# Pixie8888/R3DFSSeg

Hardware: AMD Instinct MI355X
Metric: episodes/sec S3DIS 2-way 5-shot 2048-pt (MPTI+attention, train step: forward+backward+grad all-reduce+Adam) (higher is better)
Workload: dtype f32 (index-free GEMMs -- self-attention, 1x1 convolutions, weight gradients, the EdgeConv backward's edge GEMMs -- as bf16x3 split products on the bf16 MFMA with fp32 accumulate; every index-deciding result: fp32)

## Files before the change

r3dfsseg_amd/csrc/knn.hip:

```cpp
#include <stdlib.h>
#include "common.h"

#define KNN_Q 32
#define KNN_CH 128
#define KNN_SLAB 64
#define KNN_ROWS_PER_WAVE 8

enum { R3D_SCORE_DGCNN = 0, R3D_SCORE_L2 = 1 };

__global__ void r3d_sqnorm_kernel(const float* __restrict__ x, long ldx, int rows, int C,
                                  float* __restrict__ out) {
  int i = blockIdx.x * blockDim.x + threadIdx.x;
  if (i >= rows) return;
  const float* p = x + (long)i * ldx;
  float acc = 0.f;
  for (int c = 0; c < C; ++c) acc = __builtin_fmaf(p[c], p[c], acc);
  out[i] = acc;
}

template <int R>
struct TopList {
  float v[R];
  int id[R];
};
// ... 359 lines not shown
        const unsigned long long ge = __ballot(lv[r] >= cv);
        const int p = h ? __popc((unsigned)(ge >> 32)) : __popc((unsigned)ge);
        const float upv = dpp_wave_shr1_f(lv[r]);
        const int upi = dpp_wave_shr1_i(li[r]);
        if (act) {
          if (j == p) { lv[r] = cv; li[r] = cidx; }
          else if (j > p) { lv[r] = upv; li[r] = upi; }
        }
        const float tlo = r3d_readlane_f(lv[r], klo);
        const float thi = r3d_readlane_f(lv[r], khi);
        thr[r] = h ? thi : tlo;
      }
    }
  };
  {
    int st = w;
    if (st < nsub) bload(st, bfA, njA);
    while (st < nsub) {
      const int st2 = st + 4;
      if (st2 < nsub) bload(st2, bfB, njB);
      {
        f32x16 sc;
        scores(st, bfA, njA, sc);
        select(st, sc);
      }
      st = st2;
      if (st >= nsub) break;
      const int st3 = st + 4;
      if (st3 < nsub) bload(st3, bfA, njA);
      {
        f32x16 sc;
        scores(st, bfB, njB, sc);
        select(st, sc);
      }
      st = st3;
    }
  }
  KSTAMP(3);

  __syncthreads();
  float* mv = smem;
  int* mi = (int*)(smem + 32 * 128);
#pragma unroll
  for (int r = 0; r < 16; ++r) {
    const int q = r3d_acc_row(r, lane);
    mv[(q * 4 + w) * 32 + j] = lv[r];
    mi[(q * 4 + w) * 32 + j] = li[r];
  }
  __syncthreads();
  for (int qq = 0; qq < 8; ++qq) {
    const int q = 8 * w + qq;
    const int row = q0 + q;
    if (row >= n) break;
    const float v0 = mv[q * 128 + lane], v1 = mv[q * 128 + 64 + lane];
    const int i0 = mi[q * 128 + lane], i1 = mi[q * 128 + 64 + lane];
    int rank0 = 0, rank1 = 0;
#pragma unroll
    for (int l4 = 0; l4 < 4; ++l4) {
      const float lvv = (l4 < 2) ? v0 : v1;
      const int lii = (l4 < 2) ? i0 : i1;
      const unsigned long long real = __ballot(lvv != -INFINITY);
      const int cnt = __popc((unsigned)(real >> (32 * (l4 & 1))));
      for (int t = 0; t < cnt; ++t) {
        const float ov = r3d_readlane_f(lvv, 32 * (l4 & 1) + t);
        const int oi = __builtin_amdgcn_readlane(lii, 32 * (l4 & 1) + t);
        rank0 += entry_better(ov, oi, v0, i0) ? 1 : 0;
        rank1 += entry_better(ov, oi, v1, i1) ? 1 : 0;
      }
    }
    if (v0 != -INFINITY && rank0 < k) {
      idx_out[((long)b * N + row) * k + rank0] = i0;
      if (score_out) score_out[((long)b * N + row) * k + rank0] = v0;
    }
    if (v1 != -INFINITY && rank1 < k) {
      idx_out[((long)b * N + row) * k + rank1] = i1;
      if (score_out) score_out[((long)b * N + row) * k + rank1] = v1;
    }
  }
  KSTAMP(4);
}

static __device__ __forceinline__ unsigned knn_lane_xor(unsigned v, int j, int lane) {
  const int x = (int)v;
  switch (j) {
    case 1: return (unsigned)__builtin_amdgcn_update_dpp(x, x, 0xB1, 0xF, 0xF, false);
    case 2: return (unsigned)__builtin_amdgcn_update_dpp(x, x, 0x4E, 0xF, 0xF, false);
    case 4: {
      const int t = __builtin_amdgcn_update_dpp(x, x, 0x104, 0xF, 0x5, false);
      return (unsigned)__builtin_amdgcn_update_dpp(t, x, 0x114, 0xF, 0xA, false);
    }
    case 8: return (unsigned)__builtin_amdgcn_update_dpp(x, x, 0x128, 0xF, 0xF, false);
    case 16: {
      const auto r = __builtin_amdgcn_permlane16_swap(v, v, false, false);
      return (lane & 16) ? r[0] : r[1];
    }
    default: {
      const auto r = __builtin_amdgcn_permlane32_swap(v, v, false, false);
      return (lane & 32) ? r[0] : r[1];
    }
  }
}

template <int R>
static __device__ __forceinline__ void knn_bitonic_desc(unsigned (&khi)[R], unsigned (&klo)[R], int lane) {
  static_assert(R == 1 || R == 2 || R == 4 || R == 8, "a power of two");
#pragma unroll
  for (int k = 2; k <= 64 * R; k <<= 1) {
#pragma unroll
    for (int j = k >> 1; j > 0; j >>= 1) {
      if (j >= 64) {
        const int dj = j >> 6;
#pragma unroll
        for (int i = 0; i < R; ++i) {
          if (i & dj) continue;
          const bool desc = ((64 * i) & k) == 0;
          const unsigned long long a = ((unsigned long long)khi[i] << 32) | klo[i];
          const unsigned long long b = ((unsigned long long)khi[i + dj] << 32) | klo[i + dj];
          const bool swap = desc ? a < b : a > b;
          const unsigned ah = khi[i], al = klo[i];
          khi[i] = swap ? khi[i + dj] : ah; klo[i] = swap ? klo[i + dj] : al;
          khi[i + dj] = swap ? ah : khi[i + dj]; klo[i + dj] = swap ? al : klo[i + dj];
        }
      } else {
        const bool lower = (lane & j) == 0;
#pragma unroll
        for (int i = 0; i < R; ++i) {
          const bool desc = (((64 * i) | lane) & k) == 0;
          const unsigned oh = knn_lane_xor(khi[i], j, lane), ol = knn_lane_xor(klo[i], j, lane);
          const unsigned long long a = ((unsigned long long)khi[i] << 32) | klo[i];
          const unsigned long long b = ((unsigned long long)oh << 32) | ol;
          const bool take = (lower == desc) ? b > a : b < a;
          khi[i] = take ? oh : khi[i];
          klo[i] = take ? ol : klo[i];
        }
      }
    }
  }
}

template <int KB_WAVES, int KB_CAP, int KB_TOP, int KCH ,
          int KB_SAMPLE ,
          bool FULLC ,
          int SMODE ,
          bool BFA ,
          bool BFB = false >
__global__ __launch_bounds__(64 * KB_WAVES) __attribute__((amdgpu_waves_per_eu(KB_WAVES == 4 && (FULLC || KCH < 32) ? 3 : 2)))
void r3d_knn_append_kernel(
    const float* __restrict__ xT, long ldT, int N, int C, int k, int mode, const int* __restrict__ n_dev, int n_dev_stride,
    const float* __restrict__ nrm, int* __restrict__ idx_out, float* __restrict__ score_out,
    int* __restrict__ status, int* __restrict__ tile_flags, int nsplit, int* __restrict__ idx_tmp,
    float* __restrict__ sc_tmp, const unsigned short* __restrict__ xpk ,
    const float* __restrict__ cnorm ,
    const float* __restrict__ xpm , long ldx) {
  static_assert(!BFA || (KCH == 32 && FULLC), "the bf16 threshold pass takes whole 64-channel chunks");
  static_assert(!BFB || BFA, "the bf16 filter pass shares the threshold pass's pieces");
  constexpr int KB_GROUPS = KB_WAVES * 32;
  const int z = blockIdx.z;
  extern __shared__ __attribute__((aligned(16))) float smem[];
  __shared__ int cnt_s[32];
  __shared__ float tau_s[32];
  const int lin = r3d_xcd_swizzle((int)(blockIdx.y * gridDim.x + blockIdx.x), (int)(gridDim.x * gridDim.y));
  const int b = lin / (int)gridDim.x, tile_x = lin - b * (int)gridDim.x;
  const int n = n_dev ? min(n_dev[(long)b * n_dev_stride], N) : N;
  const int q0 = tile_x * 32;
  if (q0 >= n) return;
  const int tid = threadIdx.x, lane = tid & 63, w = tid >> 6;
  const int h = lane >> 5, j = lane & 31;
  const int nch = (C + 2 * KCH - 1) / (2 * KCH);
  const int Cs = nch * 2 * KCH + (BFB ? 4 : 1);
  float* Aq = smem;
  float* region = smem + 32 * Cs;
  const float* xb = xT + (long)b * C * ldT;
  const float* nb = nrm + (long)b * N;

  for (int e = tid; e < 32 * nch * 2 * KCH; e += 64 * KB_WAVES) {
    const int c = e >> 5, jj = e & 31;
    const float v = xb[(long)min(c, C - 1) * ldT + min(q0 + jj, n - 1)];
    Aq[jj * Cs + c] = r3d_keep(v, c < C && q0 + jj < n);
  }
  if (tid < 32) cnt_s[tid] = 0;
  const int Cp = nch * 64;
  const int QRS = 2 * Cp + 8;
  unsigned short* Aqb = reinterpret_cast<unsigned short*>(region + ((32 * (KB_TOP * KB_GROUPS + 1) + 3) & ~3));
  const unsigned short* xpb = BFA ? xpk + (long)b * N * 2 * Cp : nullptr;
  if (BFA) {
    const int cpr = 2 * Cp / 8;
    for (int e = tid; e < 32 * cpr; e += 64 * KB_WAVES) {
      const int c8 = e >> 5, jj = e & 31;
      *reinterpret_cast<r3d_u32x4*>(Aqb + jj * QRS + 8 * c8) =
          *reinterpret_cast<const r3d_u32x4*>(xpb + ((long)c8 * N + min(q0 + jj, n - 1)) * 8);
    }
  }
  KSTAMP(8);
  float nq[16];
#pragma unroll
  for (int r = 0; r < 16; ++r) {
    const int row = q0 + r3d_acc_row(r, lane);
    nq[r] = r3d_keep(nb[min(row, n - 1)], row < n);
  }
  const float* cnb = BFA ? cnorm + (long)b * N : nullptr;
  const float slack = (float)(C + 8) * 0x1p-24f;
  auto bound_k = [&](int i) { return cnb[i] * (1.f + 0x1p-12f) + nb[i] * slack; };
  float* kq_s = reinterpret_cast<float*>(Aqb + 32 * QRS);
  if (BFA && tid < 32) kq_s[tid] = bound_k(min(q0 + tid, n - 1));
  auto bound_ku = [&](int i) { return cnb[i] * (1.f - 0x1p-12f) - nb[i] * slack; };
  if (BFB && tid < 32) kq_s[32 + tid] = bound_ku(min(q0 + tid, n - 1));
  __syncthreads();

  const int nsub = ((n + 31) / 32 - z + nsplit - 1) / nsplit;
  const int my_sub = (nsub - w + KB_WAVES - 1) / KB_WAVES;
  const int T = (w < nsub) ? my_sub * nch : 0;

  int stride = KB_SAMPLE;
  auto bload = [&](int t, float (&bf)[KCH]) {
    const int st = (w + KB_WAVES * stride * (t / nch)) * nsplit + z, ch = (t % nch);
    const int cand = 32 * st + j;
    const bool ok = cand < n;
    const int cc = min(cand, n - 1);
    if (FULLC) {
      const float* p = xb + (long)(2 * KCH * ch + h) * ldT + cc;
      const long st2 = 2 * ldT;
#pragma unroll
      for (int s = 0; s < KCH; ++s) bf[s] = p[s * st2];
    } else {
#pragma unroll
      for (int s = 0; s < KCH; ++s) {
        const int c = 2 * KCH * ch + 2 * s + h;
        bf[s] = r3d_keep(xb[(long)min(c, C - 1) * ldT + cc], ok && c < C);
      }
    }
  };
  f32x16 acc;
  auto mma = [&](int t, const float (&bf)[KCH]) {
    const int ch = (t % nch);
    if (ch == 0) {
#pragma unroll
      for (int r = 0; r < 16; ++r) acc[r] = 0.f;
    }
    const float* ap = Aq + j * Cs + 2 * KCH * ch + h;
    float av[KCH];
#pragma unroll
    for (int s = 0; s < KCH; ++s) av[s] = ap[2 * s];
    __builtin_amdgcn_sched_barrier(0);
#pragma unroll
    for (int s = 0; s < KCH; ++s) acc = __builtin_amdgcn_mfma_f32_32x32x2f32(av[s], bf[s], acc, 0, 0, 0);
  };
  float kb[16];
  auto load_kb = [&](int which) {
#pragma unroll
    for (int r = 0; r < 16; ++r) kb[r] = kq_s[32 * which + r3d_acc_row(r, lane)];
  };
  auto scores_lb = [&](int st, f32x16& sc) {
    const int cand = 32 * st + j;
    const float kj = bound_k(min(cand, n - 1));
#pragma unroll
    for (int r = 0; r < 16; ++r) {
      const float v = __builtin_fmaf(2.f, acc[r], -(kb[r] + kj));
      sc[r] = SMODE == R3D_SCORE_DGCNN ? v : fminf(v, 0.f);
    }
    if (32 * st + 32 > n) {
      const bool valid = cand < n;
#pragma unroll
      for (int r = 0; r < 16; ++r) sc[r] = valid ? sc[r] : -INFINITY;
    }
  };
  auto scores_ub = [&](int st, f32x16& sc) {
    const int cand = 32 * st + j;
    const float kj = bound_ku(min(cand, n - 1));
#pragma unroll
    for (int r = 0; r < 16; ++r) {
      const float v = __builtin_fmaf(2.f, acc[r], -(kb[r] + kj));
      sc[r] = SMODE == R3D_SCORE_DGCNN ? v : fminf(v, 0.f);
    }
    if (32 * st + 32 > n) {
      const bool valid = cand < n;
#pragma unroll
      for (int r = 0; r < 16; ++r) sc[r] = valid ? sc[r] : -INFINITY;
    }
  };
  auto scores = [&](int st, f32x16& sc) {
    const int cand = 32 * st + j;
    const bool valid = cand < n;
    const float nj = r3d_keep(nb[min(cand, n - 1)], valid);
#pragma unroll
    for (int r = 0; r < 16; ++r) {
      float v;
      if (SMODE == R3D_SCORE_DGCNN) {
        const float inner = -2.f * acc[r];
        v = ((-nj) - inner) - nq[r];
      } else {
        const float dis = (nq[r] + nj) - 2.f * acc[r];
        v = -fmaxf(dis, 0.f);
      }
      sc[r] = v;
    }
    if (32 * st + 32 > n) {
#pragma unroll
      for (int r = 0; r < 16; ++r) sc[r] = valid ? sc[r] : -INFINITY;
    }
  };

  float bfA[KCH], bfB[KCH];
  float g1[16], g2[16];
#pragma unroll
  for (int r = 0; r < 16; ++r) { g1[r] = -INFINITY; g2[r] = -INFINITY; }
  auto finishA_sub = [&](int i) {
    f32x16 sc;
    if (BFA) scores_lb((w + KB_WAVES * stride * i) * nsplit + z, sc);
    else scores((w + KB_WAVES * stride * i) * nsplit + z, sc);
#pragma unroll
    for (int r = 0; r < 16; ++r) {
      const float x = sc[r];
      if (KB_TOP == 2) {
        const float lo = fminf(g1[r], x);
        g2[r] = fmaxf(g2[r], lo);
      }
      g1[r] = fmaxf(g1[r], x);
    }
  };
  auto finishA = [&](int t) {
    if ((t % nch) == nch - 1) finishA_sub(t / nch);
  };
  KSTAMP(9);
  const int TA = (w < nsub) ? ((my_sub + KB_SAMPLE - 1) / KB_SAMPLE) * nch : 0;
  r3d_u32x4 pfA[8], pfB[8];
  const __amdgpu_buffer_rsrc_t rpk = __builtin_amdgcn_make_buffer_rsrc(
      (void*)(BFA ? xpb : (const unsigned short*)xT), 0, BFA ? (int)((long)N * 2 * Cp * 2) : 0, 0x00020000);
  const int chunk_b = N * 16;
  auto pload = [&](int i, int ch, r3d_u32x4 (&pf)[8]) {
    const int st = (w + KB_WAVES * stride * i) * nsplit + z;
    const int cc = min(32 * st + j, n - 1);
    const int voff = (h * N + cc) * 16;
    const int soff = 8 * ch * chunk_b, lo = (Cp / 8) * chunk_b;
#pragma unroll
    for (int s4 = 0; s4 < 4; ++s4) {
      pf[2 * s4] = __builtin_amdgcn_raw_buffer_load_b128(rpk, voff, soff + 2 * s4 * chunk_b, 0);
      pf[2 * s4 + 1] = __builtin_amdgcn_raw_buffer_load_b128(rpk, voff, soff + lo + 2 * s4 * chunk_b, 0);
    }
  };
  auto pmma = [&](int ch, const r3d_u32x4 (&pf)[8]) {
    if (ch == 0) {
#pragma unroll
      for (int r = 0; r < 16; ++r) acc[r] = 0.f;
    }
    const unsigned short* ap = Aqb + j * QRS + 64 * ch + 8 * h;
#pragma unroll
    for (int half = 0; half < 2; ++half) {
      r3d_u32x4 ah[2], al[2];
#pragma unroll
      for (int u = 0; u < 2; ++u) {
        ah[u] = *reinterpret_cast<const r3d_u32x4*>(ap + 16 * (2 * half + u));
        al[u] = *reinterpret_cast<const r3d_u32x4*>(ap + Cp + 16 * (2 * half + u));
      }
#pragma unroll
      for (int u = 0; u < 2; ++u) {
        const int s4 = 2 * half + u;
        acc = r3d_mfma_bf16(al[u], pf[2 * s4], acc);
        acc = r3d_mfma_bf16(ah[u], pf[2 * s4 + 1], acc);
        acc = r3d_mfma_bf16(ah[u], pf[2 * s4], acc);
      }
    }
  };
  auto bf_pass = [&](int n_sub, auto&& finish) {
    const int U = n_sub * nch;
    if (U <= 0) return;
    int i_c = 0, ch_c = 0, i_n = 0, ch_n = 0;
    auto advance = [&](int& i, int& ch) {
      if (++ch == nch) { ch = 0; ++i; }
    };
    pload(0, 0, pfA);
    advance(i_n, ch_n);
    int u = 0;
    for (; u + 1 < U; u += 2) {
      pload(i_n, ch_n, pfB);
      __builtin_amdgcn_sched_barrier(0);
      pmma(ch_c, pfA);
      if (ch_c == nch - 1) finish(i_c);
      i_c = i_n; ch_c = ch_n;
      advance(i_n, ch_n);
      const bool more = u + 2 < U;
      pload(more ? i_n : i_c, more ? ch_n : ch_c, pfA);
      __builtin_amdgcn_sched_barrier(0);
      pmma(ch_c, pfB);
      if (ch_c == nch - 1) finish(i_c);
      i_c = i_n; ch_c = ch_n;
      advance(i_n, ch_n);
    }
    if (u < U) {
      pmma(ch_c, pfA);
      if (ch_c == nch - 1) finish(i_c);
    }
  };
  if (BFA) {
    load_kb(0);
    bf_pass((w < nsub) ? (my_sub + KB_SAMPLE - 1) / KB_SAMPLE : 0, finishA_sub);
  } else {
    if (TA > 0) bload(0, bfB);
    for (int t = 0; t < TA; ++t) {
#pragma unroll
      for (int s = 0; s < KCH; ++s) bfA[s] = bfB[s];
      if (t + 1 < TA) bload(t + 1, bfB);
      __builtin_amdgcn_sched_barrier(0);
      mma(t, bfA);
      finishA(t);
    }
  }
  KSTAMP(10);
  stride = 1;
  {
    constexpr int GS = KB_TOP * KB_GROUPS + 1;
#pragma unroll
    for (int r = 0; r < 16; ++r) {
      const int q = r3d_acc_row(r, lane);
      region[q * GS + KB_TOP * (32 * w + j)] = g1[r];
      if (KB_TOP == 2) region[q * GS + 2 * (32 * w + j) + 1] = g2[r];
    }
    __syncthreads();
    for (int qq = 0; qq < 32 / KB_WAVES; ++qq) {
      const int q = (32 / KB_WAVES) * w + qq;
      unsigned key[KB_TOP * KB_GROUPS / 64];
#pragma unroll
      for (int i = 0; i < KB_TOP * KB_GROUPS / 64; ++i) key[i] = f2key(region[q * GS + 64 * i + lane]) >> 16;
      unsigned res = 0;
      for (int bit = 15; bit >= 0; --bit) {
        const unsigned cand = res | (1u << bit);
        int c = 0;
#pragma unroll
        for (int i = 0; i < KB_TOP * KB_GROUPS / 64; ++i) c += __popcll(__ballot(key[i] >= cand));
        if (c >= k) res = cand;
      }
      if (lane == 0) tau_s[q] = key2f(res << 16);
    }
    __syncthreads();
  }
  KSTAMP(11);
  float tauq[16];
#pragma unroll
  for (int r = 0; r < 16; ++r) tauq[r] = q0 + r3d_acc_row(r, lane) < n ? tau_s[r3d_acc_row(r, lane)] : INFINITY;
  __syncthreads();

  static_assert(!BFB || 32 * KB_CAP <= 32 * (KB_TOP * KB_GROUPS + 1), "the index buffer must end in front of the query pieces");
  float* bufv = region + (BFB ? 32 * KB_CAP : 0);
  int* bufi = (int*)(region + (BFB ? 0 : 32 * KB_CAP));
  constexpr bool BMP = BFB && KB_WAVES == 4;
  unsigned* bm = reinterpret_cast<unsigned*>(region);
  bool overflow = false;
  auto finishB = [&](int t) {
    if ((t % nch) != nch - 1) return;
    const int st = (w + KB_WAVES * (t / nch)) * nsplit + z;
    f32x16 sc;
    scores(st, sc);
#pragma unroll
    for (int r = 0; r < 16; ++r) {
      if (sc[r] >= tauq[r]) {
        const int q = r3d_acc_row(r, lane);
        const int slot = atomicAdd(&cnt_s[q], 1);
        if (slot < KB_CAP) {
          bufv[q * KB_CAP + slot] = sc[r];
          bufi[q * KB_CAP + slot] = 32 * st + j;
        } else {
          overflow = true;
        }
      }
    }
  };
  auto finishBF = [&](int i) {
    const int st = (w + KB_WAVES * i) * nsplit + z;
    f32x16 sc;
    scores_ub(st, sc);
    if (BMP) {
      unsigned long long m[16];
#pragma unroll
      for (int r = 0; r < 16; ++r) m[r] = __ballot(sc[r] >= tauq[r]);
      __builtin_amdgcn_sched_barrier(0);
      int word = 0;
#define KB_LO(r) "s"((int)(unsigned)(m[r] & 0xffffffffull))
#define KB_HI(r) "s"((int)(unsigned)(m[r] >> 32))
      asm volatile(
                   "s_nop 4\n\t"
                   "v_writelane_b32 %0, %1, 0\n\t"
                   "v_writelane_b32 %0, %2, 4\n\t"
                   "v_writelane_b32 %0, %3, 1\n\t"
                   "v_writelane_b32 %0, %4, 5\n\t"
                   "v_writelane_b32 %0, %5, 2\n\t"
                   "v_writelane_b32 %0, %6, 6\n\t"
                   "v_writelane_b32 %0, %7, 3\n\t"
                   "v_writelane_b32 %0, %8, 7\n\t"
                   "v_writelane_b32 %0, %9, 8\n\t"
                   "v_writelane_b32 %0, %10, 12\n\t"
                   "v_writelane_b32 %0, %11, 9\n\t"
                   "v_writelane_b32 %0, %12, 13\n\t"
                   "v_writelane_b32 %0, %13, 10\n\t"
                   "v_writelane_b32 %0, %14, 14\n\t"
                   "v_writelane_b32 %0, %15, 11\n\t"
                   "v_writelane_b32 %0, %16, 15"
                   : "+v"(word)
                   : KB_LO(0), KB_HI(0), KB_LO(1), KB_HI(1), KB_LO(2), KB_HI(2), KB_LO(3), KB_HI(3), KB_LO(4), KB_HI(4), KB_LO(5), KB_HI(5), KB_LO(6), KB_HI(6), KB_LO(7), KB_HI(7));
      asm volatile(
                   "s_nop 4\n\t"
                   "v_writelane_b32 %0, %1, 16\n\t"
                   "v_writelane_b32 %0, %2, 20\n\t"
                   "v_writelane_b32 %0, %3, 17\n\t"
                   "v_writelane_b32 %0, %4, 21\n\t"
                   "v_writelane_b32 %0, %5, 18\n\t"
                   "v_writelane_b32 %0, %6, 22\n\t"
                   "v_writelane_b32 %0, %7, 19\n\t"
                   "v_writelane_b32 %0, %8, 23\n\t"
                   "v_writelane_b32 %0, %9, 24\n\t"
                   "v_writelane_b32 %0, %10, 28\n\t"
                   "v_writelane_b32 %0, %11, 25\n\t"
                   "v_writelane_b32 %0, %12, 29\n\t"
                   "v_writelane_b32 %0, %13, 26\n\t"
                   "v_writelane_b32 %0, %14, 30\n\t"
                   "v_writelane_b32 %0, %15, 27\n\t"
                   "v_writelane_b32 %0, %16, 31"
                   : "+v"(word)
                   : KB_LO(8), KB_HI(8), KB_LO(9), KB_HI(9), KB_LO(10), KB_HI(10), KB_LO(11), KB_HI(11), KB_LO(12), KB_HI(12), KB_LO(13), KB_HI(13), KB_LO(14), KB_HI(14), KB_LO(15), KB_HI(15));
#undef KB_LO
#undef KB_HI
      __builtin_amdgcn_sched_barrier(0);
      const int ls = w + KB_WAVES * i;
      if (lane < 32) bm[ls * 32 + ((lane + ls) & 31)] = (unsigned)word;
      return;
    }
#pragma unroll
    for (int r = 0; r < 16; ++r) {
      if (sc[r] >= tauq[r]) {
        const int q = r3d_acc_row(r, lane);
        const int slot = atomicAdd(&cnt_s[q], 1);
        if (slot < KB_CAP) bufi[q * KB_CAP + slot] = 32 * st + j;
        else overflow = true;
      }
    }
  };
  if (BFB) {
    load_kb(1);
    bf_pass((w < nsub) ? my_sub : 0, finishBF);
  } else {
    if (T > 0) bload(0, bfB);
    for (int t = 0; t < T; ++t) {
#pragma unroll
      for (int s = 0; s < KCH; ++s) bfA[s] = bfB[s];
      if (t + 1 < T) bload(t + 1, bfB);
      __builtin_amdgcn_sched_barrier(0);
      mma(t, bfA);
      finishB(t);
    }
  }
  KSTAMP(12);
  if (BMP) {
    __syncthreads();
    constexpr int QW = 32 / KB_WAVES, NCH = (KB_CAP + 63) / 64;
    unsigned wq[QW][NCH];
#pragma unroll
    for (int i = 0; i < QW; ++i)
#pragma unroll
      for (int cch = 0; cch < NCH; ++cch) {
        const int ls = 64 * cch + lane;
        wq[i][cch] = ls < nsub ? bm[ls * 32 + ((QW * w + i + ls) & 31)] : 0u;
      }
    __syncthreads();
#pragma unroll
    for (int i = 0; i < QW; ++i) {
      const int q = QW * w + i;
      int total = 0;
#pragma unroll
      for (int cch = 0; cch < NCH; ++cch) {
        if (64 * cch >= nsub) break;
        unsigned word = wq[i][cch];
        const int c = __popc(word);
        const int incl = r3d_wave_incl_scan(c);
        int off = total + incl - c;
        const int cand0 = 32 * ((64 * cch + lane) * nsplit + z);
        while (word) {
          const int bit = __ffs((int)word) - 1;
          if (off < KB_CAP) bufi[q * KB_CAP + off] = cand0 + bit;
          ++off;
          word &= word - 1;
        }
        total += __builtin_amdgcn_readlane(incl, 63);
      }
      if (lane == 0) cnt_s[q] = total;
      overflow = overflow || total > KB_CAP;
    }
  }
  if (__any(overflow) && lane == 0) {
    if (status) atomicOr(status, 1);
    if (tile_flags) tile_flags[(long)b * gridDim.x + tile_x] = 1;
  }
  __syncthreads();
  if (BFA && tid < 32 && q0 + tid < n && cnt_s[tid] < min(k, n)) {
    if (status) atomicOr(status, 2);
    if (tile_flags) tile_flags[(long)b * gridDim.x + tile_x] = 1;
  }
  KSTAMP(14);

  if (BFB) {
    constexpr int QW = 32 / KB_WAVES;
    int off[QW + 1];
    off[0] = 0;
#pragma unroll
    for (int i = 0; i < QW; ++i) off[i + 1] = off[i] + __builtin_amdgcn_readfirstlane(min(cnt_s[QW * w + i], KB_CAP));
    const int total = off[QW];
    const int nseg = C / 32;
    const int T2 = ((total + 63) / 64) * nseg;
    int q_cur = 0, slot_cur = 0;
    bool ok_cur = false;
    const float4* xr_cur = nullptr;
    auto locate = [&](int t, int& q, int& slot, bool& ok, const float4*& xr) {
      const int f = 64 * (t / nseg) + lane;
      ok = f < total;
      int ql = 0;
#pragma unroll
      for (int i = 1; i < QW; ++i) ql += f >= off[i] ? 1 : 0;
      ql = ok ? ql : 0;
      q = QW * w + ql;
      slot = ok ? f - off[ql] : 0;
      const int cand = min(max(bufi[q * KB_CAP + slot], 0), n - 1);
      xr = reinterpret_cast<const float4*>(xpm + ((long)b * N + cand) * ldx) + 8 * (t % nseg);
    };
    float4 xa[8], xb[8];
    int qn = 0, slotn = 0;
    bool okn = false;
    const float4* xrn = nullptr;
    if (T2 > 0) {
      locate(0, q_cur, slot_cur, ok_cur, xr_cur);
#pragma unroll
      for (int u = 0; u < 8; ++u) xa[u] = xr_cur[u];
    }
    float a = 0.f;
    for (int t = 0; t < T2; ++t) {
      const int tn = min(t + 1, T2 - 1);
      locate(tn, qn, slotn, okn, xrn);
#pragma unroll
      for (int u = 0; u < 8; ++u) xb[u] = xrn[u];
      __builtin_amdgcn_sched_barrier(0);
      const int sg = t % nseg;
      if (sg == 0) a = 0.f;
      const float4* aq = reinterpret_cast<const float4*>(Aq + q_cur * Cs + 32 * sg);
      float4 qa[8];
#pragma unroll
      for (int u = 0; u < 8; ++u) qa[u] = aq[u];
#pragma unroll
      for (int u = 0; u < 8; ++u) {
        a = __builtin_fmaf(qa[u].x, xa[u].x, a);
        a = __builtin_fmaf(qa[u].y, xa[u].y, a);
        a = __builtin_fmaf(qa[u].z, xa[u].z, a);
        a = __builtin_fmaf(qa[u].w, xa[u].w, a);
      }
      if (sg == nseg - 1 && ok_cur) {
        const int cand = min(max(bufi[q_cur * KB_CAP + slot_cur], 0), n - 1);
        const float nj = nb[cand], nqq = nb[min(q0 + q_cur, n - 1)];
        float v;
        if (SMODE == R3D_SCORE_DGCNN) {
          const float inner = -2.f * a;
          v = ((-nj) - inner) - nqq;
        } else {
          const float dis = (nqq + nj) - 2.f * a;
          v = -fmaxf(dis, 0.f);
        }
        bufv[q_cur * KB_CAP + slot_cur] = v;
      }
#pragma unroll
      for (int u = 0; u < 8; ++u) xa[u] = xb[u];
      q_cur = qn; slot_cur = slotn; ok_cur = okn;
    }
  }
  KSTAMP(15);
  for (int qq = 0; qq < 32 / KB_WAVES; ++qq) {
    const int q = (32 / KB_WAVES) * w + qq;
    const int row = q0 + q;
    if (row >= n) break;
    const int M = __builtin_amdgcn_readfirstlane(min(cnt_s[q], KB_CAP));
    float mv[KB_CAP / 64];
    int mi[KB_CAP / 64], rank[KB_CAP / 64];
    unsigned khi[KB_CAP / 64], klo[KB_CAP / 64];
    unsigned long long key[KB_CAP / 64];
#pragma unroll
    for (int i = 0; i < KB_CAP / 64; ++i) {
      const int e = 64 * i + lane;
      mi[i] = e < M ? bufi[q * KB_CAP + e] : 0x7fffffff;
      mv[i] = e < M ? bufv[q * KB_CAP + e] : -INFINITY;
      khi[i] = f2key(mv[i] + 0.0f);
      klo[i] = 0x7fffffffu - (unsigned)mi[i];
      key[i] = ((unsigned long long)khi[i] << 32) | klo[i];
      rank[i] = 0;
    }
    bool sorted = false;
    if constexpr (KB_CAP >= 256) {
    if (M > 64 && N <= (1 << 22)) {
      constexpr int RMAX = KB_CAP > 256 ? 8 : 4;
      static_assert(64 * RMAX >= KB_CAP && KB_CAP <= 512, "the slot field of a sort key has 9 bits");
      unsigned sh[RMAX], sl[RMAX];
#pragma unroll
      for (int i = 0; i < RMAX; ++i) {
        const int e = 64 * i + lane;
        const bool in = i < KB_CAP / 64 && e < M;
        sh[i] = in ? khi[i < KB_CAP / 64 ? i : 0] : 0u;
        sl[i] = in ? ((0x3fffffu - (unsigned)mi[i < KB_CAP / 64 ? i : 0]) << 9) | (unsigned)e : 0u;
      }
      if (M <= 256) {
        unsigned h4[4] = {sh[0], sh[1], sh[2], sh[3]}, l4[4] = {sl[0], sl[1], sl[2], sl[3]};
        knn_bitonic_desc<4>(h4, l4, lane);
#pragma unroll
        for (int i = 0; i < 4; ++i) sl[i] = l4[i];
      } else {
        knn_bitonic_desc<RMAX>(sh, sl, lane);
      }
#pragma unroll
      for (int i = 0; i < KB_CAP / 64; ++i) {
        const int e = 64 * i + lane;
        const int slot = (int)(sl[i] & 511u);
        const bool out = e < M;
        mi[i] = out ? bufi[q * KB_CAP + slot] : 0x7fffffff;
        mv[i] = out ? bufv[q * KB_CAP + slot] : -INFINITY;
        rank[i] = e;
      }
      sorted = true;
    }
    }
    if (sorted) {
    } else if (M <= 64) {
#pragma unroll 4
      for (int t = 0; t < M; ++t) {
        const unsigned long long ok = ((unsigned long long)(unsigned)__builtin_amdgcn_readlane((int)khi[0], t) << 32) |
                                      (unsigned)__builtin_amdgcn_readlane((int)klo[0], t);
        rank[0] += ok > key[0] ? 1 : 0;
      }
    } else {
#pragma unroll
      for (int c = 0; c < KB_CAP / 64; ++c) {
        const int cnt = min(max(M - 64 * c, 0), 64);
#pragma unroll 4
        for (int t = 0; t < cnt; ++t) {
          const unsigned long long ok = ((unsigned long long)(unsigned)__builtin_amdgcn_readlane((int)khi[c], t) << 32) |
                                        (unsigned)__builtin_amdgcn_readlane((int)klo[c], t);
#pragma unroll
          for (int i = 0; i < KB_CAP / 64; ++i) rank[i] += ok > key[i] ? 1 : 0;
        }
      }
    }
    if (nsplit == 1) {
#pragma unroll
      for (int i = 0; i < KB_CAP / 64; ++i) {
        if (64 * i + lane < M && rank[i] < k) {
          idx_out[((long)b * N + row) * k + rank[i]] = mi[i];
          if (score_out) score_out[((long)b * N + row) * k + rank[i]] = mv[i];
        }
      }
    } else {
      const long o = (((long)z * gridDim.y + b) * N + row) * k;
#pragma unroll
      for (int i = 0; i < KB_CAP / 64; ++i) {
        if (64 * i + lane < M && rank[i] < k) {
          idx_tmp[o + rank[i]] = mi[i];
          sc_tmp[o + rank[i]] = mv[i];
        }
      }
      for (int t = min(M, k) + lane; t < k; t += 64) {
        idx_tmp[o + t] = 0x7fffffff;
        sc_tmp[o + t] = -INFINITY;
      }
    }
  }
  KSTAMP(13);
}

__global__ __launch_bounds__(256) void r3d_knn_merge_kernel(const int* __restrict__ idx_tmp, const float* __restrict__ sc_tmp,
                                                            int nsplit, long rows, int k, const int* __restrict__ n_dev, int n_dev_stride, int N,
                                                            int* __restrict__ idx_out, float* __restrict__ score_out) {
  __shared__ unsigned long long keys[4][2][256];
  const int lane = threadIdx.x & 63, w = threadIdx.x >> 6;
  const long row = (long)blockIdx.x * 4 + w;
  if (row >= rows) return;
  if (n_dev && (int)(row % N) >= min(n_dev[(row / N) * n_dev_stride], N)) return;
  for (int p = 0; p < 2; ++p)
    for (int t = lane; t < k; t += 64) {
      const long o = ((long)p * rows + row) * k + t;
      const float v = sc_tmp[o];
      const int id = idx_tmp[o];
      keys[w][p][t] = id == 0x7fffffff ? 0ull
                                       : (((unsigned long long)f2key(v + 0.0f) << 32) | (0x7fffffffu - (unsigned)id));
    }
  __builtin_amdgcn_wave_barrier();
  for (int p = 0; p < 2; ++p)
    for (int t = lane; t < k; t += 64) {
      const unsigned long long mine = keys[w][p][t];
      if (mine == 0ull) continue;
      const unsigned long long* other = keys[w][1 - p];
      int lo = 0, hi = k;
      while (lo < hi) {
        const int mid = (lo + hi) >> 1;
        if (other[mid] > mine) lo = mid + 1; else hi = mid;
      }
      const int rank = t + lo;
      if (rank < k) {
        const long o = ((long)p * rows + row) * k + t;
        idx_out[row * k + rank] = idx_tmp[o];
        if (score_out) score_out[row * k + rank] = sc_tmp[o];
      }
    }
}

__global__ __launch_bounds__(1024) void r3d_knn_mean_kernel(const float* __restrict__ x, long ldx, int N, int C,
                                                            const int* __restrict__ n_dev, int n_dev_stride, int Cp,
                                                            float* __restrict__ mean ) {
  __shared__ float part[16][64];
  const int b = blockIdx.y, c = blockIdx.x * 64 + (threadIdx.x & 63), ph = threadIdx.x >> 6;
  const int n = n_dev ? min(n_dev[(long)b * n_dev_stride], N) : N;
  float s = 0.f;
  if (c < C) {
    const float* p = x + (long)b * N * ldx + c;
    int r = ph;
    for (; r + 7 * 16 < n; r += 8 * 16) {
      float v[8];
#pragma unroll
      for (int u = 0; u < 8; ++u) v[u] = p[(long)(r + 16 * u) * ldx];
#pragma unroll
      for (int u = 0; u < 8; ++u) s += v[u];
    }
    for (; r < n; r += 16) s += p[(long)r * ldx];
  }
  part[ph][threadIdx.x & 63] = s;
  __syncthreads();
  if (ph == 0 && c < Cp) {
    float t = 0.f;
#pragma unroll
    for (int q = 0; q < 16; ++q) t += part[q][threadIdx.x];
    mean[(long)b * Cp + c] = c < C && n > 0 ? t / (float)n : 0.f;
  }
}
__global__ void r3d_knn_pack_bf_kernel(const float* __restrict__ x, long ldx, long rows, int N, int C, int Cp,
                                       const float* __restrict__ mean, unsigned short* __restrict__ out) {
  const long i = (long)blockIdx.x * blockDim.x + threadIdx.x;
  const int cpr = Cp / 8;
  if (i >= rows * cpr) return;
  const long m = i / cpr;
  const int c8 = (int)(i - m * cpr);
  const long set = m / N;
  const int pt = (int)(m - set * N);
  const int c0 = 8 * c8;
  const float* mu = mean + set * Cp + c0;
  float v[8];
#pragma unroll
  for (int u = 0; u < 8; ++u) v[u] = r3d_keep(x[m * ldx + min(c0 + u, C - 1)] - mu[u], c0 + u < C);
  const r3d_bx3 f = r3d_bx3_split8(v);
  unsigned short* o = out + set * N * 2 * Cp;
  *reinterpret_cast<r3d_u32x4*>(o + ((long)c8 * N + pt) * 8) = f.h;
  *reinterpret_cast<r3d_u32x4*>(o + ((long)(cpr + c8) * N + pt) * 8) = f.m;
}
__global__ __launch_bounds__(256) void r3d_knn_cnorm_kernel(const float* __restrict__ x, long ldx, long rows, int N, int C, int Cp,
                                                            const float* __restrict__ mean, float* __restrict__ cnorm) {
  const int lane = threadIdx.x & 63, sub = lane & 15;
  const long m = ((long)blockIdx.x * 4 + (threadIdx.x >> 6)) * 4 + (lane >> 4);
  const long mc = m < rows ? m : rows - 1;
  const float* mu = mean + (mc / N) * Cp;
  float s = 0.f;
  if ((ldx & 3) == 0 && (C & 3) == 0 && ((uintptr_t)x & 15) == 0) {
    for (int c = 4 * sub; c < C; c += 64) {
      const float4 v = *reinterpret_cast<const float4*>(x + mc * ldx + c), u = *reinterpret_cast<const float4*>(mu + c);
      const float d0 = v.x - u.x, d1 = v.y - u.y, d2 = v.z - u.z, d3 = v.w - u.w;
      s = __builtin_fmaf(d0, d0, s); s = __builtin_fmaf(d1, d1, s); s = __builtin_fmaf(d2, d2, s); s = __builtin_fmaf(d3, d3, s);
    }
  } else {
    for (int c = sub; c < C; c += 16) {
      const float d = x[mc * ldx + c] - mu[c];
      s = __builtin_fmaf(d, d, s);
    }
  }
  s += __int_as_float(__builtin_amdgcn_mov_dpp(__float_as_int(s), 0xB1, 0xF, 0xF, true));
  s += __int_as_float(__builtin_amdgcn_mov_dpp(__float_as_int(s), 0x4E, 0xF, 0xF, true));
  s += __int_as_float(__builtin_amdgcn_mov_dpp(__float_as_int(s), 0x141, 0xF, 0xF, true));
  s += __int_as_float(__builtin_amdgcn_mov_dpp(__float_as_int(s), 0x140, 0xF, 0xF, true));
  if (sub == 0 && m < rows) cnorm[m] = s;
}
static int g_knn_bf16_threshold = getenv("R3D_KNN_FP32_THRESHOLD") ? 0 : 1;
static int g_knn_bf16_filter = getenv("R3D_KNN_FP32_PASS_B") ? 0 : 1;
extern "C" int r3d_debug_set_knn_bf16_filter(int on) {
  const int old = g_knn_bf16_filter;
  g_knn_bf16_filter = on > 0 ? 1 : 0;
  return old;
}
extern "C" int r3d_debug_set_knn_bf16_threshold(int on) {
  const int old = g_knn_bf16_threshold;
  g_knn_bf16_threshold = on ? 1 : 0;
  return old;
}
#ifndef KM_WAVES
#define KM_WAVES 4
#define KM_CAP 128
#define KM_TOP 1
#endif
#ifndef KM_SAMPLE
#define KM_SAMPLE 2
#endif

static size_t knn_append_lds_bytes(int C, int waves, int cap, int top, int kch, bool bfa) {
  const int nch = (C + 2 * kch - 1) / (2 * kch);
  const size_t a = 32 * (size_t)(nch * 2 * kch + 4);
  size_t g = 32 * (size_t)(top * waves * 32 + 1);
  if (bfa) g = ((g + 3) & ~(size_t)3) + 32 * (size_t)(2 * nch * 64 + 8) / 2 + 64;
  const size_t bsz = 2 * 32 * (size_t)cap;
  return sizeof(float) * (a + (g > bsz ? g : bsz));
}
static size_t knn_lds_bytes(int C) {
  const int Cp = (C + 1) & ~1;
  return sizeof(float) * ((size_t)KNN_Q * (Cp + 1) + (size_t)KNN_CH * (KNN_SLAB + 1) +
                          (size_t)KNN_Q * (KNN_CH + 1) + KNN_Q);
}

extern "C" int r3d_sqnorm(const float* x, long ldx, long rows, int C, float* out, void* stream) {
  R3D_REQUIRE(x && out && rows > 0 && C > 0 && ldx >= C, "r3d_sqnorm: bad arguments");
  hipLaunchKernelGGL(r3d_sqnorm_kernel, dim3(r3d_cdiv(rows, 256)), dim3(256), 0, (hipStream_t)stream, x,
                     ldx, (int)rows, C, out);
  R3D_LAUNCH_CHECK("r3d_sqnorm");
  return R3D_OK;
}

extern "C" int r3d_pm_to_cm_pitched(const float* in, long ld, int B, int C, int N, float* out, long pitch, void* stream);
extern "C" long r3d_cm_pitch(int N) { return (long)((N + 31) / 32) * 32 + 32; }
extern "C" long r3d_knn_norm_ws_words(int B, int N) { return (long)B * N + (long)B * ((N + 31) / 32) + 64; }

enum KnnPath {
  KNN_STREAMED_SMALL,
  KNN_STREAMED_LARGE,
  KNN_INSERTION,
};
struct KnnPlan {
  KnnPath path;
  bool few;
  bool split;
  bool bf;
  long norms, tile_flags, xcm, pieces, mean, cnorm, split_idx, split_sc, words;
};
static KnnPlan knn_plan(int B, int N, int C, int k, bool status, bool x_cm, bool extras) {
  KnnPlan p = {};
  const long tiles = ((long)N + 31) / 32;
  if (k <= 32 && C <= 64) {
    p.path = KNN_STREAMED_SMALL;
    p.few = tiles * B <= 256;
    p.bf = extras && C % 64 == 0 && !p.few;
  } else if (status && knn_append_lds_bytes(C, 8, 384, 2, 32, false) <= 160 * 1024) {
    p.path = KNN_STREAMED_LARGE;
    p.split = extras && 2 * tiles * B <= 256 && N >= 4L * k;
    p.bf = extras && !p.split && C % 64 == 0 && knn_append_lds_bytes(C, 8, 384, 2, 32, true) <= 160 * 1024;
  } else {
    p.path = KNN_INSERTION;
  }
  long at = 0;
  auto part = [&](long words) {
    const long o = at;
    at += (words + 63) / 64 * 64;
    return o;
  };
  p.norms = part((long)B * N);
  p.tile_flags = part(p.path == KNN_STREAMED_SMALL ? B * tiles : 0);
  p.xcm = part(p.path != KNN_INSERTION && !x_cm ? (long)B * C * r3d_cm_pitch(N) : 0);
  p.pieces = part(p.bf ? (long)B * N * C : 0);
  p.mean = part(p.bf ? (long)B * C : 0);
  p.cnorm = part(p.bf ? (long)B * N : 0);
  p.split_idx = part(p.split ? 2L * B * N * k : 0);
  p.split_sc = part(p.split ? 2L * B * N * k : 0);
  p.words = at;
  return p;
}

extern "C" long r3d_knn_ws_words(int B, int N, int C, int k, int flags) {
  return knn_plan(B, N, C, k, flags & 1, flags & 2, true).words;
}

struct KnnCall {
  const float* x; long ldx; const float* xT; long ldT;
  int B, N, C, k, mode; const int* n_dev; int n_stride; int32_t* idx; float* sc; hipStream_t st;
  float *norms; int* tile_flags; float* cm; unsigned short* pieces; float *mean, *cnorm; int* split_idx; float* split_sc;
};

template <int WAVES, int CAP, int TOP, int KCH, int SAMPLE, bool FULLC, bool BFA = false, bool BFB = false>
static int knn_append_launch(const KnnCall& c, dim3 grid, int* status, int* tile_flags) {
  const size_t lds = knn_append_lds_bytes(c.C, WAVES, CAP, TOP, KCH, BFA);
  auto go = [&](auto smode) {
    constexpr int SM = decltype(smode)::value;
    static size_t attr = 0;
    if (lds > attr) {
      hipError_t e = hipFuncSetAttribute((const void*)r3d_knn_append_kernel<WAVES, CAP, TOP, KCH, SAMPLE, FULLC, SM, BFA, BFB>,
                                         hipFuncAttributeMaxDynamicSharedMemorySize, (int)lds);
      R3D_REQUIRE(e == hipSuccess, "r3d_knn_topk: cannot reserve %zu B of LDS: %s", lds, hipGetErrorString(e));
      attr = lds;
    }
    hipLaunchKernelGGL((r3d_knn_append_kernel<WAVES, CAP, TOP, KCH, SAMPLE, FULLC, SM, BFA, BFB>), grid, dim3(64 * WAVES), lds,
                       c.st, c.xT, c.ldT, c.N, c.C, c.k, SM, c.n_dev, c.n_stride, c.norms, c.idx, c.sc, status, tile_flags,
                       (int)grid.z, c.split_idx, c.split_sc, BFA ? c.pieces : nullptr, BFA ? c.cnorm : nullptr,
                       BFB ? c.x : nullptr, c.ldx);
    return R3D_OK;
  };
  return c.mode == R3D_SCORE_DGCNN ? go(std::integral_constant<int, R3D_SCORE_DGCNN>())
                                   : go(std::integral_constant<int, R3D_SCORE_L2>());
}

template <int R>
static void knn_insertion_launch(const KnnCall& c, size_t lds) {
  static bool attr_set = false;
  if (!attr_set) {
    hipFuncSetAttribute((const void*)r3d_knn_topk_kernel<R>, hipFuncAttributeMaxDynamicSharedMemorySize, 160 * 1024);
    attr_set = true;
  }
  hipLaunchKernelGGL(r3d_knn_topk_kernel<R>, dim3(r3d_cdiv(c.N, KNN_Q), c.B), dim3(256), lds, c.st, c.x, c.ldx, c.N, c.C,
                     c.k, c.mode, c.n_dev, c.n_stride, c.norms, c.idx, c.sc);
}

static int knn_cm_operand(KnnCall& c, const float* x_cm) {
  c.xT = x_cm;
  c.ldT = c.N;
  if (!x_cm) {
    R3D_REQUIRE(c.cm && c.x, "r3d_knn_topk: need x_cm or (x and cm_ws)");
    c.ldT = r3d_cm_pitch(c.N);
    int rc = r3d_pm_to_cm_pitched(c.x, c.ldx, c.B, c.C, c.N, c.cm, c.ldT, c.st);
    if (rc) return rc;
    c.xT = c.cm;
  }
  hipLaunchKernelGGL(r3d_sqnorm_cm_kernel, dim3(r3d_cdiv(c.N, 256), c.B), dim3(256), 0, c.st, c.xT, c.ldT, c.C, c.N, c.norms);
  return R3D_OK;
}

static void knn_pack_bf(const KnnCall& c) {
  const long rows = (long)c.B * c.N;
  hipLaunchKernelGGL(r3d_knn_mean_kernel, dim3(c.C / 64, c.B), dim3(1024), 0, c.st, c.x, c.ldx, c.N, c.C, c.n_dev, c.n_stride,
                     c.C, c.mean);
  hipLaunchKernelGGL(r3d_knn_pack_bf_kernel, dim3(r3d_cdiv(rows * (c.C / 8), 256)), dim3(256), 0, c.st, c.x, c.ldx, rows, c.N,
                     c.C, c.C, c.mean, c.pieces);
  hipLaunchKernelGGL(r3d_knn_cnorm_kernel, dim3(r3d_cdiv(rows, 16)), dim3(256), 0, c.st, c.x, c.ldx, rows, c.N, c.C, c.C,
                     c.mean, c.cnorm);
}

static int knn_topk_impl(const float* x, long ldx, const float* x_cm, int B, int N, int C, int k, int mode,
                         const int* n_valid_dev, int n_valid_stride, float* ws, long ws_words, float* norm_ws, float* cm_ws,
                         int32_t* idx_out, float* score_out, int32_t* status, void* stream) {
  R3D_REQUIRE((x || x_cm) && (ws || norm_ws) && idx_out, "r3d_knn_topk: null pointer");
  R3D_REQUIRE(B > 0 && N > 0 && C > 0 && (!x || ldx >= C), "r3d_knn_topk: bad shape B=%d N=%d C=%d ldx=%ld", B, N, C, ldx);
  R3D_REQUIRE(k > 0 && k <= N && k <= 256, "r3d_knn_topk: unsupported k=%d (need 1..min(N,256))", k);
  R3D_REQUIRE(mode == R3D_SCORE_DGCNN || mode == R3D_SCORE_L2, "r3d_knn_topk: unknown mode %d", mode);
  const KnnPlan p = knn_plan(B, N, C, k, status, x_cm, ws);
  KnnCall c = {x, ldx, nullptr, 0, B, N, C, k, mode, n_valid_dev, n_valid_stride, idx_out, score_out, (hipStream_t)stream};
  if (ws) {
    R3D_REQUIRE(((uintptr_t)ws & 15) == 0 && ws_words >= p.words,
                "r3d_knn_topk_batched: ws must be 16-byte aligned and hold r3d_knn_ws_words = %ld floats (got %ld)", p.words,
                ws_words);
    c.norms = ws + p.norms;
    c.tile_flags = (int*)(ws + p.tile_flags);
    c.cm = ws + p.xcm;
    c.pieces = (unsigned short*)(ws + p.pieces);
    c.mean = ws + p.mean;
    c.cnorm = ws + p.cnorm;
    c.split_idx = (int*)(ws + p.split_idx);
    c.split_sc = ws + p.split_sc;
  } else {
    c.norms = norm_ws;
    c.tile_flags = (int*)(norm_ws + (long)B * N);
    c.cm = cm_ws;
  }
  if (p.path == KNN_INSERTION) {
    R3D_REQUIRE(c.x, "r3d_knn_topk: the insertion kernel needs the point-major matrix");
    const size_t lds = knn_lds_bytes(c.C);
    R3D_REQUIRE(lds <= 160 * 1024, "r3d_knn_topk: C=%d needs %zu B of LDS (> 160 KiB)", c.C, lds);
    int rc = r3d_sqnorm(c.x, c.ldx, (long)c.B * c.N, c.C, c.norms, c.st);
    if (rc) return rc;
    if (c.k <= 64) knn_insertion_launch<1>(c, lds);
    else if (c.k <= 128) knn_insertion_launch<2>(c, lds);
    else knn_insertion_launch<4>(c, lds);
    R3D_LAUNCH_CHECK("r3d_knn_topk");
    return R3D_OK;
  }
  int rc = knn_cm_operand(c, x_cm);
  if (rc) return rc;
  const bool bfa = p.bf && g_knn_bf16_threshold && c.x;
  const dim3 grid(r3d_cdiv(c.N, 32), c.B);
  if (p.path == KNN_STREAMED_SMALL) {
    r3d_zero_words(c.tile_flags, (long)c.B * grid.x, c.st);
    if (c.C <= 16) {
      rc = p.few ? knn_append_launch<8, KM_CAP, KM_TOP, 8, KM_SAMPLE, false>(c, grid, nullptr, c.tile_flags)
                 : knn_append_launch<KM_WAVES, KM_CAP, KM_TOP, 8, KM_SAMPLE, false>(c, grid, nullptr, c.tile_flags);
    } else if (bfa) {
      knn_pack_bf(c);
      const bool filter = g_knn_bf16_filter && (c.ldx & 3) == 0 && ((uintptr_t)c.x & 15) == 0 && grid.x <= KM_CAP;
      rc = filter ? knn_append_launch<KM_WAVES, KM_CAP, KM_TOP, 32, 1, true, true, true>(c, grid, nullptr, c.tile_flags)
                  : knn_append_launch<KM_WAVES, KM_CAP, KM_TOP, 32, KM_SAMPLE, true, true>(c, grid, nullptr, c.tile_flags);
    } else if (c.C % 64 == 0) {
      rc = p.few ? knn_append_launch<8, KM_CAP, KM_TOP, 32, KM_SAMPLE, true>(c, grid, nullptr, c.tile_flags)
                 : knn_append_launch<KM_WAVES, KM_CAP, KM_TOP, 32, KM_SAMPLE, true>(c, grid, nullptr, c.tile_flags);
    } else {
      rc = p.few ? knn_append_launch<8, KM_CAP, KM_TOP, 32, KM_SAMPLE, false>(c, grid, nullptr, c.tile_flags)
                 : knn_append_launch<KM_WAVES, KM_CAP, KM_TOP, 32, KM_SAMPLE, false>(c, grid, nullptr, c.tile_flags);
    }
    if (rc) return rc;
    hipLaunchKernelGGL(c.C <= 16 ? r3d_knn_small_kernel<8> : r3d_knn_small_kernel<32>, grid, dim3(256), 0, c.st, c.xT, c.ldT, c.N,
                       c.C, c.k, c.mode, c.n_dev, c.n_stride, c.norms, c.idx, c.sc, (const int*)c.tile_flags);
    R3D_LAUNCH_CHECK("r3d_knn_topk(small)");
    return R3D_OK;
  }
  r3d_zero_words(status, 1, c.st);
  const dim3 gb(grid.x, c.B, p.split ? 2 : 1);
  if (bfa) {
    knn_pack_bf(c);
    rc = knn_append_launch<8, 384, 2, 32, 1, true, true>(c, gb, status, nullptr);
  } else if (c.C % 64 == 0) {
    rc = knn_append_launch<8, 384, 2, 32, 1, true>(c, gb, status, nullptr);
  } else {
    rc = knn_append_launch<8, 384, 2, 32, 1, false>(c, gb, status, nullptr);
  }
  if (rc) return rc;
  if (p.split)
    hipLaunchKernelGGL(r3d_knn_merge_kernel, dim3(r3d_cdiv((long)c.B * c.N, 4)), dim3(256), 0, c.st, c.split_idx, c.split_sc, 2,
                       (long)c.B * c.N, c.k, c.n_dev, c.n_stride, c.N, c.idx, c.sc);
  R3D_LAUNCH_CHECK("r3d_knn_topk(big)");
  return R3D_OK;
}

extern "C" int r3d_knn_topk(const float* x, long ldx, const float* x_cm, int B, int N, int C, int k, int mode,
                            const int* n_valid_dev, float* norm_ws, float* cm_ws, int32_t* idx_out,
                            float* score_out, int32_t* status, void* stream) {
  return knn_topk_impl(x, ldx, x_cm, B, N, C, k, mode, n_valid_dev, 0, nullptr, 0, norm_ws, cm_ws, idx_out, score_out, status,
                       stream);
}

extern "C" int r3d_knn_topk_batched(const float* x, long ldx, const float* x_cm, int B, int N, int C, int k, int mode,
                                    const int* n_valid_dev, int n_valid_stride, float* ws, long ws_words, int32_t* idx_out,
                                    float* score_out, int32_t* status, void* stream) {
  R3D_REQUIRE(n_valid_stride >= 0, "r3d_knn_topk_batched: negative stride");
  return knn_topk_impl(x, ldx, x_cm, B, N, C, k, mode, n_valid_dev, n_valid_stride, ws, ws_words, nullptr, nullptr, idx_out,
                       score_out, status, stream);
}
```

Before: 387.3.

## Extend bf16 MFMA threshold-and-filter KNN path to small channel counts

Generalizes the bf16 split-product threshold pass to a 16-channel chunk (KCH=8) and adds an fp32 exact-rescoring filter pass for C<=16. The small-channel KNN (e.g. xyz-space neighbours) now packs padded bf16 pieces and runs MFMA-based candidate thresholding instead of the fp32 append path. The aim is to cut the fp32 score cost in the first EdgeConv layer. In exchange it adds the pack, mean and cnorm launches plus a register-pipelined candidate rescoring loop, and the results depend on the candidate caps not overflowing.

```diff
diff --git a/r3dfsseg_amd/csrc/knn.hip b/r3dfsseg_amd/csrc/knn.hip
--- a/r3dfsseg_amd/csrc/knn.hip
+++ b/r3dfsseg_amd/csrc/knn.hip
@@ -535,7 +535,8 @@
     float* __restrict__ sc_tmp, const unsigned short* __restrict__ xpk ,
     const float* __restrict__ cnorm ,
     const float* __restrict__ xpm , long ldx) {
-  static_assert(!BFA || (KCH == 32 && FULLC), "the bf16 threshold pass takes whole 64-channel chunks");
+  static_assert(!BFA || (KCH == 32 && FULLC) || (KCH == 8 && BFB && KB_WAVES == 4 && KB_TOP == 1),
+                "the bf16 threshold pass takes whole 64-channel chunks, or one 16-channel chunk with the filter");
   static_assert(!BFB || BFA, "the bf16 filter pass shares the threshold pass's pieces");
   constexpr int KB_GROUPS = KB_WAVES * 32;
   const int z = blockIdx.z;
@@ -562,7 +563,8 @@
     Aq[jj * Cs + c] = r3d_keep(v, c < C && q0 + jj < n);
   }
   if (tid < 32) cnt_s[tid] = 0;
-  const int Cp = nch * 64;
+  constexpr int S4 = KCH / 8;
+  const int Cp = nch * 2 * KCH;
   const int QRS = 2 * Cp + 8;
   unsigned short* Aqb = reinterpret_cast<unsigned short*>(region + ((32 * (KB_TOP * KB_GROUPS + 1) + 3) & ~3));
   const unsigned short* xpb = BFA ? xpk + (long)b * N * 2 * Cp : nullptr;
@@ -706,38 +708,39 @@
   };
   KSTAMP(9);
   const int TA = (w < nsub) ? ((my_sub + KB_SAMPLE - 1) / KB_SAMPLE) * nch : 0;
-  r3d_u32x4 pfA[8], pfB[8];
+  r3d_u32x4 pfA[2 * S4], pfB[2 * S4];
   const __amdgpu_buffer_rsrc_t rpk = __builtin_amdgcn_make_buffer_rsrc(
       (void*)(BFA ? xpb : (const unsigned short*)xT), 0, BFA ? (int)((long)N * 2 * Cp * 2) : 0, 0x00020000);
   const int chunk_b = N * 16;
-  auto pload = [&](int i, int ch, r3d_u32x4 (&pf)[8]) {
+  auto pload = [&](int i, int ch, r3d_u32x4 (&pf)[2 * S4]) {
     const int st = (w + KB_WAVES * stride * i) * nsplit + z;
     const int cc = min(32 * st + j, n - 1);
     const int voff = (h * N + cc) * 16;
-    const int soff = 8 * ch * chunk_b, lo = (Cp / 8) * chunk_b;
-#pragma unroll
-    for (int s4 = 0; s4 < 4; ++s4) {
+    const int soff = 2 * S4 * ch * chunk_b, lo = (Cp / 8) * chunk_b;
+#pragma unroll
+    for (int s4 = 0; s4 < S4; ++s4) {
       pf[2 * s4] = __builtin_amdgcn_raw_buffer_load_b128(rpk, voff, soff + 2 * s4 * chunk_b, 0);
       pf[2 * s4 + 1] = __builtin_amdgcn_raw_buffer_load_b128(rpk, voff, soff + lo + 2 * s4 * chunk_b, 0);
     }
   };
-  auto pmma = [&](int ch, const r3d_u32x4 (&pf)[8]) {
+  auto pmma = [&](int ch, const r3d_u32x4 (&pf)[2 * S4]) {
     if (ch == 0) {
 #pragma unroll
       for (int r = 0; r < 16; ++r) acc[r] = 0.f;
     }
-    const unsigned short* ap = Aqb + j * QRS + 64 * ch + 8 * h;
-#pragma unroll
-    for (int half = 0; half < 2; ++half) {
-      r3d_u32x4 ah[2], al[2];
-#pragma unroll
-      for (int u = 0; u < 2; ++u) {
-        ah[u] = *reinterpret_cast<const r3d_u32x4*>(ap + 16 * (2 * half + u));
-        al[u] = *reinterpret_cast<const r3d_u32x4*>(ap + Cp + 16 * (2 * half + u));
-      }
-#pragma unroll
-      for (int u = 0; u < 2; ++u) {
-        const int s4 = 2 * half + u;
+    const unsigned short* ap = Aqb + j * QRS + 2 * KCH * ch + 8 * h;
+    constexpr int U2 = S4 < 2 ? S4 : 2;
+#pragma unroll
+    for (int half = 0; half < S4 / U2; ++half) {
+      r3d_u32x4 ah[U2], al[U2];
+#pragma unroll
+      for (int u = 0; u < U2; ++u) {
+        ah[u] = *reinterpret_cast<const r3d_u32x4*>(ap + 16 * (U2 * half + u));
+        al[u] = *reinterpret_cast<const r3d_u32x4*>(ap + Cp + 16 * (U2 * half + u));
+      }
+#pragma unroll
+      for (int u = 0; u < U2; ++u) {
+        const int s4 = U2 * half + u;
         acc = r3d_mfma_bf16(al[u], pf[2 * s4], acc);
         acc = r3d_mfma_bf16(ah[u], pf[2 * s4 + 1], acc);
         acc = r3d_mfma_bf16(ah[u], pf[2 * s4], acc);
@@ -978,7 +981,73 @@
   }
   KSTAMP(14);
 
-  if (BFB) {
+  if constexpr (BFB && KCH == 8) {
+    constexpr int QW = 32 / KB_WAVES;
+    int off[QW + 1];
+    off[0] = 0;
+#pragma unroll
+    for (int i = 0; i < QW; ++i) off[i + 1] = off[i] + __builtin_amdgcn_readfirstlane(min(cnt_s[QW * w + i], KB_CAP));
+    const int total = off[QW];
+    const int T2 = (total + 63) / 64;
+    auto locate = [&](int t, int& q, int& slot, bool& ok, int& cand) {
+      const int f = 64 * t + lane;
+      ok = f < total;
+      int ql = 0;
+#pragma unroll
+      for (int i = 1; i < QW; ++i) ql += f >= off[i] ? 1 : 0;
+      ql = ok ? ql : 0;
+      q = QW * w + ql;
+      slot = ok ? f - off[ql] : 0;
+      cand = min(max(bufi[q * KB_CAP + slot], 0), n - 1);
+    };
+    auto rload = [&](int cand, float (&v)[16]) {
+      const float* xr = xpm + ((long)b * N + cand) * ldx;
+#pragma unroll
+      for (int c = 0; c < 16; ++c) v[c] = r3d_keep(xr[min(c, C - 1)], c < C);
+    };
+    int q_cur = 0, slot_cur = 0, cand_cur = 0;
+    bool ok_cur = false;
+    float xa[16], xn[16];
+    if (T2 > 0) {
+      locate(0, q_cur, slot_cur, ok_cur, cand_cur);
+      rload(cand_cur, xa);
+    }
+    for (int t = 0; t < T2; ++t) {
+      int qn, slotn, candn;
+      bool okn;
+      locate(min(t + 1, T2 - 1), qn, slotn, okn, candn);
+      rload(candn, xn);
+      __builtin_amdgcn_sched_barrier(0);
+      const float4* aq = reinterpret_cast<const float4*>(Aq + q_cur * Cs);
+      float4 qa[4];
+#pragma unroll
+      for (int u = 0; u < 4; ++u) qa[u] = aq[u];
+      float a = 0.f;
+#pragma unroll
+      for (int u = 0; u < 4; ++u) {
+        a = __builtin_fmaf(qa[u].x, xa[4 * u], a);
+        a = __builtin_fmaf(qa[u].y, xa[4 * u + 1], a);
+        a = __builtin_fmaf(qa[u].z, xa[4 * u + 2], a);
+        a = __builtin_fmaf(qa[u].w, xa[4 * u + 3], a);
+      }
+      if (ok_cur) {
+        const float nj = nb[cand_cur], nqq = nb[min(q0 + q_cur, n - 1)];
+        float v;
+        if (SMODE == R3D_SCORE_DGCNN) {
+          const float inner = -2.f * a;
+          v = ((-nj) - inner) - nqq;
+        } else {
+          const float dis = (nqq + nj) - 2.f * a;
+          v = -fmaxf(dis, 0.f);
+        }
+        bufv[q_cur * KB_CAP + slot_cur] = v;
+      }
+#pragma unroll
+      for (int c = 0; c < 16; ++c) xa[c] = xn[c];
+      q_cur = qn; slot_cur = slotn; cand_cur = candn; ok_cur = okn;
+    }
+  }
+  if constexpr (BFB && KCH == 32) {
     constexpr int QW = 32 / KB_WAVES;
     int off[QW + 1];
     off[0] = 0;
@@ -1278,11 +1347,13 @@
 #define KM_SAMPLE 2
 #endif
 
+static int knn_piece_channels(int C) { return C <= 16 ? 16 : C; }
+
 static size_t knn_append_lds_bytes(int C, int waves, int cap, int top, int kch, bool bfa) {
   const int nch = (C + 2 * kch - 1) / (2 * kch);
   const size_t a = 32 * (size_t)(nch * 2 * kch + 4);
   size_t g = 32 * (size_t)(top * waves * 32 + 1);
-  if (bfa) g = ((g + 3) & ~(size_t)3) + 32 * (size_t)(2 * nch * 64 + 8) / 2 + 64;
+  if (bfa) g = ((g + 3) & ~(size_t)3) + 32 * (size_t)(2 * nch * 2 * kch + 8) / 2 + 64;
   const size_t bsz = 2 * 32 * (size_t)cap;
   return sizeof(float) * (a + (g > bsz ? g : bsz));
 }
@@ -1322,7 +1393,7 @@
   if (k <= 32 && C <= 64) {
     p.path = KNN_STREAMED_SMALL;
     p.few = tiles * B <= 256;
-    p.bf = extras && C % 64 == 0 && !p.few;
+    p.bf = extras && (C % 64 == 0 || C <= 16) && !p.few;
   } else if (status && knn_append_lds_bytes(C, 8, 384, 2, 32, false) <= 160 * 1024) {
     p.path = KNN_STREAMED_LARGE;
     p.split = extras && 2 * tiles * B <= 256 && N >= 4L * k;
@@ -1339,8 +1410,8 @@
   p.norms = part((long)B * N);
   p.tile_flags = part(p.path == KNN_STREAMED_SMALL ? B * tiles : 0);
   p.xcm = part(p.path != KNN_INSERTION && !x_cm ? (long)B * C * r3d_cm_pitch(N) : 0);
-  p.pieces = part(p.bf ? (long)B * N * C : 0);
-  p.mean = part(p.bf ? (long)B * C : 0);
+  p.pieces = part(p.bf ? (long)B * N * knn_piece_channels(C) : 0);
+  p.mean = part(p.bf ? (long)B * knn_piece_channels(C) : 0);
   p.cnorm = part(p.bf ? (long)B * N : 0);
   p.split_idx = part(p.split ? 2L * B * N * k : 0);
   p.split_sc = part(p.split ? 2L * B * N * k : 0);
@@ -1407,11 +1478,12 @@
 
 static void knn_pack_bf(const KnnCall& c) {
   const long rows = (long)c.B * c.N;
-  hipLaunchKernelGGL(r3d_knn_mean_kernel, dim3(c.C / 64, c.B), dim3(1024), 0, c.st, c.x, c.ldx, c.N, c.C, c.n_dev, c.n_stride,
-                     c.C, c.mean);
-  hipLaunchKernelGGL(r3d_knn_pack_bf_kernel, dim3(r3d_cdiv(rows * (c.C / 8), 256)), dim3(256), 0, c.st, c.x, c.ldx, rows, c.N,
-                     c.C, c.C, c.mean, c.pieces);
-  hipLaunchKernelGGL(r3d_knn_cnorm_kernel, dim3(r3d_cdiv(rows, 16)), dim3(256), 0, c.st, c.x, c.ldx, rows, c.N, c.C, c.C,
+  const int Cp = knn_piece_channels(c.C);
+  hipLaunchKernelGGL(r3d_knn_mean_kernel, dim3(r3d_cdiv(Cp, 64), c.B), dim3(1024), 0, c.st, c.x, c.ldx, c.N, c.C, c.n_dev,
+                     c.n_stride, Cp, c.mean);
+  hipLaunchKernelGGL(r3d_knn_pack_bf_kernel, dim3(r3d_cdiv(rows * (Cp / 8), 256)), dim3(256), 0, c.st, c.x, c.ldx, rows, c.N,
+                     c.C, Cp, c.mean, c.pieces);
+  hipLaunchKernelGGL(r3d_knn_cnorm_kernel, dim3(r3d_cdiv(rows, 16)), dim3(256), 0, c.st, c.x, c.ldx, rows, c.N, c.C, Cp,
                      c.mean, c.cnorm);
 }
 
@@ -1459,7 +1531,10 @@
   const dim3 grid(r3d_cdiv(c.N, 32), c.B);
   if (p.path == KNN_STREAMED_SMALL) {
     r3d_zero_words(c.tile_flags, (long)c.B * grid.x, c.st);
-    if (c.C <= 16) {
+    if (c.C <= 16 && bfa && g_knn_bf16_filter && grid.x <= KM_CAP) {
+      knn_pack_bf(c);
+      rc = knn_append_launch<4, KM_CAP, 1, 8, 1, false, true, true>(c, grid, nullptr, c.tile_flags);
+    } else if (c.C <= 16) {
       rc = p.few ? knn_append_launch<8, KM_CAP, KM_TOP, 8, KM_SAMPLE, false>(c, grid, nullptr, c.tile_flags)
                  : knn_append_launch<KM_WAVES, KM_CAP, KM_TOP, 8, KM_SAMPLE, false>(c, grid, nullptr, c.tile_flags);
     } else if (bfa) {
```

Result: faster. 391.5, median of 6 (+1.1%).
